# felixyu7/perceiver-io-1

Hardware: AMD Instinct MI355X
Metric: samples/sec (whole node) IMDB MLM seq_len=512 at 1/2/4/8 MI355X (higher is better)
Workload: dtype bf16; 1 GPU; mlm256; model=perceiver-io-mlm latents=256x64 layers=3x(1+6) vocab=10003, global_batch=64, seq_len=512, parallelism=dp1, backend=hip, graph=True, allreduce_in_graph=False, bucket_update=False

## Files before the change

perceiver_io_amd/csrc/binding.cpp:

```cpp
#include <torch/extension.h>
#include <ATen/hip/HIPContext.h>
#include <hip/hip_runtime.h>

#include "host_api.h"

#include <unordered_map>
#include <vector>

using torch::Tensor;
using OptT = c10::optional<Tensor>;

namespace {
hipStream_t stream() { return at::hip::getCurrentHIPStream(); }

#ifndef PIO_CHECKS
#define PIO_CHECKS 0
#endif
int64_t check_errors(bool reset) {
  return (int64_t)(pio::check_errors_elementwise(reset) | pio::check_errors_optim(reset) |
                   pio::check_errors_mlm_head(reset) | pio::check_errors_ce_head(reset) | pio::check_errors_topk_head(reset) |
                   pio::check_errors_rowgemm(reset) | pio::check_errors_pixel_head(reset) |
                   pio::check_errors_soft_ce_head(reset) | pio::check_errors_augment(reset) |
                   pio::check_errors_randaugment(reset) | pio::check_errors_health(reset) |
                   pio::check_errors_lartpc_prep(reset));
// ... 1365 lines not shown
}

Tensor embed_fwd(Tensor ids, Tensor E, Tensor P, double scale) {
  TORCH_CHECK(ids.is_contiguous() && E.is_contiguous() && P.is_contiguous());
  CHECK_DT(ids, torch::kInt64);
  const long long rows = ids.numel();
  const int L = (int)ids.size(1), C = (int)E.size(1);
  TORCH_CHECK(C % 4 == 0, "embedding width must be a multiple of 4");
  Tensor out = torch::empty({ids.size(0), L, C}, E.options());
  pio::embed_fwd_launch(ids.data_ptr<int64_t>(), f32p(E), f32p(P), out.data_ptr<float>(), rows, L, C, (float)scale,
                        E.size(0), stream());
  checked_sync("embed_fwd");
  return out;
}

void embed_bwd(Tensor ids, Tensor g, OptT dE, OptT dP, double scale, OptT job_slab, std::vector<Tensor> job_dsts,
               std::vector<int64_t> job_offs) {
  TORCH_CHECK(g.is_contiguous() && ids.is_contiguous());
  const pio::SlabJob job = make_job(job_slab, job_dsts, job_offs);
  const int B = (int)ids.size(0), L = (int)ids.size(1), C = (int)g.size(2);
  if (dE.has_value()) TORCH_CHECK(dE->is_contiguous() && dE->size(1) == C, "dE must be (V, C) contiguous");
  if (dP.has_value()) TORCH_CHECK(dP->is_contiguous() && dP->size(1) == C && dP->size(0) >= L, "dP must be (>= L, C)");
  if ((!dE.has_value() || dE->size(0) < (1 << 24)) &&
      pio::embed_bwd_local_launch(ids.data_ptr<int64_t>(), f32p(g), dE.has_value() ? dE->data_ptr<float>() : nullptr,
                                  dP.has_value() ? dP->data_ptr<float>() : nullptr, B, L, C, (float)scale, job,
                                  stream()))
    return;
  if (job.slab) pio::slab_reduce_launch(job, stream());
  if (dE.has_value()) {
    TORCH_CHECK(dE->is_contiguous() && dE->size(1) == C, "dE must be (V, C) contiguous");
// ... 827 lines not shown
        py::arg("w2"), py::arg("g2"), py::arg("be2"), py::arg("H"), py::arg("pa_grads"),
        py::arg("job_slab") = py::none(), py::arg("job_dsts") = std::vector<Tensor>(),
        py::arg("job_offs") = std::vector<int64_t>(), py::arg("seed") = py::none(), py::arg("site") = 0,
        py::arg("p") = 0.0, py::arg("zero_out") = py::none(), py::arg("att_qkv") = py::none(),
        py::arg("att_lse") = py::none(), py::arg("att_out") = py::none(), py::arg("att_scale") = 0.0);
  m.def("post_attn_bwd", &post_attn_bwd, py::arg("dz"), py::arg("y"), py::arg("m2"), py::arg("r2"), py::arg("u"),
        py::arg("o"), py::arg("wo"), py::arg("w1"), py::arg("w2"), py::arg("g2"), py::arg("be2"), py::arg("H"),
        py::arg("grads"), py::arg("slab") = false, py::arg("job_slab") = py::none(),
        py::arg("job_dsts") = std::vector<Tensor>(), py::arg("job_offs") = std::vector<int64_t>(),
        py::arg("seed") = py::none(), py::arg("site") = 0, py::arg("p") = 0.0, py::arg("zero_out") = py::none());
  m.def("ln_linear_bwd", &ln_linear_bwd, py::arg("g"), py::arg("w"), py::arg("x"), py::arg("mean"), py::arg("rstd"),
        py::arg("lnw"), py::arg("lnb"), py::arg("dres"), py::arg("need_dx"), py::arg("dlnw"), py::arg("dlnb"),
        py::arg("dW"), py::arg("db"), py::arg("pe") = py::none(), py::arg("kin") = -1, py::arg("slab") = false,
        py::arg("job_slab") = py::none(), py::arg("job_dsts") = std::vector<Tensor>(),
        py::arg("job_offs") = std::vector<int64_t>(), py::arg("dx_out") = py::none(), py::arg("pe_index") = py::none());
  m.def("wgrad", &wgrad, py::arg("g"), py::arg("a"), py::arg("amode"), py::arg("mean"), py::arg("rstd"), py::arg("lnw"),
        py::arg("lnb"), py::arg("rows_per_wg"), py::arg("dW"), py::arg("db"), py::arg("pe") = py::none(),
        py::arg("kin") = -1, py::arg("pe_index") = py::none());
  m.def("mlm_select", &mlm_select, py::arg("labels"), py::arg("cap"), py::arg("gcap"), py::arg("sticky") = py::none(),
        py::arg("queries") = py::none());
  m.def("index_add_rows", &index_add_rows);
  m.def("gather_rows", &gather_rows, py::arg("src"), py::arg("idx"));
  m.def("batch_sum2", &batch_sum2, py::arg("a"), py::arg("b"), py::arg("ob_acc") = py::none());
  m.def("pixel_ce_fwd", &pixel_ce_fwd);
  m.def("pixel_ce_bwd", &pixel_ce_bwd);
  m.def("pixel_predict", &pixel_predict, py::arg("h"), py::arg("w"), py::arg("b"), py::arg("qidx"), py::arg("qvalid"),
        py::arg("Q"), py::arg("npix"), py::arg("labels") = py::none());
  m.def("nonzero_compact", &nonzero_compact, py::arg("img"), py::arg("cap"), py::arg("segs") = 0, py::arg("tile") = 0);
  m.def("event_compact", &event_compact, py::arg("img"), py::arg("lab"), py::arg("words"), py::arg("key_cap"),
        py::arg("query_cap"), py::arg("wmask"), py::arg("ncls"), py::arg("segs") = 0, py::arg("tile") = 0);
// ... 76 lines not shown
```

perceiver_io_amd/csrc/host_api.h:

```cpp
#pragma once
#include <stdint.h>

#include <hip/hip_runtime_api.h>

namespace pio {


struct AttnArgs {
  const uint16_t* q; long long q_bs; int q_rs;
  const uint16_t* k; long long k_bs; int k_rs;
  const uint16_t* v; long long v_bs; int v_rs;
  const uint8_t* kmask;
  int B, H, Nq, Nk;
  float scale_log2;
  float scale;
  uint32_t drop_thresh;
  float drop_scale;
  const int64_t* seedp;
  uint32_t site;
};

struct DropCfg {
  const int64_t* seed;
  uint32_t site;
// ... 93 lines not shown
  RowsOut Y;
  float *mean, *rstd;
  PeSplit ps;
};
struct LnLinearBwdArgs {
  RowsIn G; int N;
  const uint16_t* W; int w_rs, Kin;
  RowsIn X;
  const float *mean, *rstd, *lnw, *lnb;
  const float* dres; int dres_rs;
  float* dX; int dx_rs;
  float *dlnw, *dlnb, *dW, *db;
  int vrs, wrs, slab;
  int R;
  PeSplit ps;
  SlabJob job;
};
struct WgradArgs {
  RowsIn G; int N;
  RowsIn A; int Kin, amode;
  const float *mean, *rstd, *lnw, *lnb;
  int R;
  int rows_per_wg;
  float *dW, *db;
  int vrs, wrs;
  PeSplit ps;
};
struct PostAttnFwdArgs {
  const uint16_t* O;
  const float* X;
// ... 194 lines not shown
                          uint8_t* classes, float* conf, uint8_t* cmap, int* cpart, hipStream_t st);
void nonzero_compact_launch(const float* img, int B, long long npix, long long cap, int S, int V, int* segcount,
                            float* values, int64_t* index, bool* kmask, int* count, hipStream_t st);
unsigned check_errors_pixel_head(bool reset);
void rand_augment_launch(const uint8_t* src, const float* words, uint8_t* out, uint8_t* tmp, int* hist, int B, int H,
                         int W, int C, int N, int fill, hipStream_t st);
unsigned check_errors_randaugment(bool reset);
void ln_linear_fwd_launch(const LnLinearFwdArgs& a, hipStream_t st);
void post_attn_fwd_launch(const PostAttnFwdArgs& a, int C, hipStream_t st);
void post_attn_ln_linear_fwd_launch(const PostAttnFwdArgs& a, int C, hipStream_t st);
bool sa_layer_fwd_launch(const SaLayerFwdArgs& a, hipStream_t st);
void post_attn_bwd_launch(const PostAttnBwdArgs& a, int C, hipStream_t st);
bool ln_linear_post_attn_bwd_launch(const LnLinearPostAttnBwdArgs& a, int C, hipStream_t st);
void ln_linear_bwd_launch(const LnLinearBwdArgs& a, hipStream_t st);
void wgrad_launch(const WgradArgs& a, hipStream_t st);
unsigned check_errors_rowgemm(bool reset);
bool sb_fwd_launch(const SBFwdArgs& a, int C, hipStream_t st);
bool sb_bwd_launch(const SBBwdArgs& a, int C, hipStream_t st);
bool sb_wgrad_launch(SBWgradArgs a, int C, const SlabJob& sj, hipStream_t st);
int soft_ce_row_tiles(int M);
void soft_ce_fwd_launch(int C, const float* Hm, const uint16_t* W, const float* bias, const int64_t* la,
                        const int64_t* lb, const float* lam, float eps, int M, int V, float* lse, int* pred,
                        uint16_t* hs, float* blk, float* loss, float* count, hipStream_t st);
void soft_ce_bwd_launch(int C, const uint16_t* Hs, const uint16_t* W, const float* bias, const int64_t* la,
                        const int64_t* lb, const float* lam, float eps, const float* lse, const float* gout,
                        const float* count, int M, int V, float* dH, float* dW, float* db, int accumulate,
                        hipStream_t st);
void batch_mix_launch(const float* x, const int64_t* y, const float* mix, float* out, int64_t* yb, float* lam_out, int B,
                      int H, int W, int Ch, hipStream_t st);
unsigned check_errors_soft_ce_head(bool reset);
// ... 9 lines not shown
```

perceiver_io_amd/csrc/rowgemm.hip:

```cpp
#include "common.h"

namespace pio {

__device__ __forceinline__ float ldf(const float* p) { return *p; }
__device__ __forceinline__ float ldf(const uint16_t* p) { return bf2f(*p); }
__device__ __forceinline__ void stf(float* p, float v) { *p = v; }
__device__ __forceinline__ void stf(uint16_t* p, float v) { *p = f2bf(v); }

template <int MAXT, bool A_KC, bool B_KC>
__device__ __forceinline__ void tile_gemm(const uint16_t* sA, int lda, const uint16_t* sB, int ldb, int BM, int BN,
                                          int K, f32x16 (&acc)[MAXT]) {
  const int w = wave_id();
  const int ntn = BN / 32, nt = (BM / 32) * ntn;
#pragma unroll
  for (int t = 0; t < MAXT; ++t) {
    const int tg = w + 4 * t;
    if (tg < nt) {
      const int m0 = 32 * (tg / ntn), n0 = 32 * (tg % ntn);
      for (int k0 = 0; k0 < K; k0 += 16) {
        const bf16x8 a = A_KC ? frag_kc(sA, lda, m0, k0) : frag_ks(sA, lda, m0, k0);
        const bf16x8 b = B_KC ? frag_kc(sB, ldb, n0, k0) : frag_ks(sB, ldb, n0, k0);
        acc[t] = mfma32(a, b, acc[t]);
      }
    }
// ... 318 lines not shown
    }
  }
}
__device__ __forceinline__ void g_store(const float (&v)[2][8], uint16_t* sG, int ldg) {
#pragma unroll
  for (int i = 0; i < 2; ++i) {
    bf16x8 b;
#pragma unroll
    for (int e = 0; e < 8; ++e) b[e] = (short)f2bf(v[i][e]);
    *reinterpret_cast<bf16x8*>(sG + ((threadIdx.x >> 3) + 32 * i) * ldg + (threadIdx.x & 7) * 8) = b;
  }
}

template <int NCH>
constexpr int ln_linear_fwd_smem() { return 2 * 64 * (32 * NCH + 8) * 2 + 64 * 68 * 4; }

template <typename TOut, int NCH, bool AV>
__device__ __forceinline__ void ln_linear_fwd_tile(float (&xv)[NCH][8], bf16x8 (&wb)[NCH], const float (&gw)[NCH][8],
                                                   const float (&gb)[NCH][8], bool has_ln, int m0, int R, int Kin,
                                                   float eps, const uint16_t* __restrict__ W, int w_rs,
                                                   const float* __restrict__ bias, int N, int act,
                                                   const float* __restrict__ res, int res_rs, TOut* __restrict__ Y,
                                                   int y_rs, float* __restrict__ mean_out, float* __restrict__ rstd_out,
                                                   uint16_t* smem, int part = 0, int nparts = 1, bool wv = false) {
  constexpr int KP = 32 * NCH, LD = KP + 8, LDO = 64 + 4;
  uint16_t* sA = smem;
  uint16_t* sW = sA + 64 * LD;
  float* sO = reinterpret_cast<float*>(sW + 64 * LD);
  const int gr = m0 + rp_row(), w = wave_id(), l = lane_id();
  const bool wvec = AV || wv;
  const int wk = w_rs > Kin ? w_rs : Kin;
  const bool yvec = (N & 7) == 0 && (y_rs & 7) == 0 && aligned16(Y);
  if (has_ln) {
    float s = 0.f;
#pragma unroll
    for (int j = 0; j < NCH; ++j)
#pragma unroll
      for (int e = 0; e < 8; ++e) s += xv[j][e];
    const float mean = quad_sum(s) / Kin;
    float q = 0.f;
#pragma unroll
    for (int j = 0; j < NCH; ++j)
#pragma unroll
      for (int e = 0; e < 8; ++e) {
        const float d = rp_col(j) + e < Kin ? xv[j][e] - mean : 0.f;
        q += d * d;
      }
    const float rstd = rsqrtf(quad_sum(q) / Kin + eps);
    if ((threadIdx.x & 3) == 0 && gr < R && mean_out && part == nparts - 1) { mean_out[gr] = mean; rstd_out[gr] = rstd; }
#pragma unroll
    for (int j = 0; j < NCH; ++j)
#pragma unroll
      for (int e = 0; e < 8; ++e) xv[j][e] = (xv[j][e] - mean) * rstd * gw[j][e] + gb[j][e];
  }
  lds_row_write_bf16<NCH>(sA, LD, xv);

  for (int n0 = 64 * part; n0 < N; n0 += 64 * nparts) {
    tile_store<NCH>(wb, sW, LD, 64, KP);
    lds_sync();
    if (n0 + 64 * nparts < N) tile_fetch<NCH>(wb, W, w_rs, n0 + 64 * nparts, N, 64, wk, KP, wvec);
    const int bc = n0 + 32 * (w & 1) + (l & 31);
    const float bv = (bias && bc < N) ? bias[bc] : 0.f;
    f32x16 acc[1] = {f32x16{}};
    tile_gemm<1, true, true>(sA, LD, sW, LD, 64, 64, KP, acc);
    for_acc<1>(64, 64, [&](int t, int m, int n, int i) {
      float v = acc[t][i] + bv;
      if (act == 1) v = gelu_f(v);
      sO[m * LDO + n] = v;
// ... 505 lines not shown
  post_attn_bwd_body<C, AV>(dz, Ysave, mean2, rstd2, U, O, Wo, W1, W2, g2, be2, dY, dO, delta, H, gr_out, R, dr, smem,
                            (int)blockIdx.y, (int)gridDim.y);
}

template <int NCH>
constexpr int ln_linear_bwd_loop_smem() {
  return 64 * 72 * 2 + 2 * 64 * (32 * NCH + 8) * 2 > 64 * (32 * NCH + 4) * 4
             ? 64 * 72 * 2 + 2 * 64 * (32 * NCH + 8) * 2
             : 64 * (32 * NCH + 4) * 4;
}
template <int NCH>
constexpr int ln_linear_bwd_smem() {
  return ln_linear_bwd_loop_smem<NCH>() + 8 * 32 * NCH * 4 + 4 * 64 * 4;
}

template <typename TG, typename TX, int NCH, bool AV>
__device__ __forceinline__ void ln_linear_bwd_body(
    const TG* __restrict__ G, int g_rs, int N, const uint16_t* __restrict__ W, int w_rs, int Kin,
    const TX* __restrict__ X,
    int x_rs, const float* __restrict__ mean, const float* __restrict__ rstd, const float* __restrict__ lnw,
    const float* __restrict__ lnb, const float* __restrict__ dres, int dres_rs, float* __restrict__ dX, int dx_rs,
    float* __restrict__ dlnw, float* __restrict__ dlnb, float* __restrict__ dW, float* __restrict__ db, int vrs,
    int wrs, int slab, int R, PeSplit ps, uint16_t* smem, float (&dxo)[NCH][8], int part = 0, int nparts = 1,
    int vf = 0) {
  const bool own_rows = tile_part_owner(3, nparts) == part;
  constexpr int KP = 32 * NCH, LD = KP + 8, LDG = 64 + 8, LDF = KP + 4;
  uint16_t* sG = smem;
  uint16_t* sW = sG + 64 * LDG;
  uint16_t* sXn = sW + 64 * LD;
  float* sF = reinterpret_cast<float*>(smem);
// ... 25 lines not shown
#pragma unroll
        for (int e = 0; e < 8; ++e) xn[j][e] += (xv[j][e] - mu) * rs * gw[j][e];
    } else {
#pragma unroll
      for (int j = 0; j < NCH; ++j)
#pragma unroll
        for (int e = 0; e < 8; ++e) xn[j][e] = xv[j][e];
    }
    lds_row_write_bf16<NCH>(sXn, LD, xn);
  }

  constexpr int MAXT = 3;
  f32x16 acc[MAXT];
#pragma unroll
  for (int t = 0; t < MAXT; ++t) acc[t] = f32x16{};
  for (int nc = 0; nc < N; nc += 64) {
    g_store(gv, sG, LDG);
    tile_store<NCH>(wb, sW, LD, 64, KP);
    float cs[8];
#pragma unroll
    for (int e = 0; e < 8; ++e) cs[e] = gv[0][e] + gv[1][e];
    lds_sync();
    if (nc + 64 < N) {
      g_fetch<TG>(gv, G, g_rs, m0, R, nc + 64, N, gvec);
      tile_fetch<NCH>(wb, W, w_rs, nc + 64, N, 64, wk, KP, wvec);
    }
    tile_gemm<MAXT, true, false>(sG, LDG, sW, LD, 64, KP, 64, acc);
    const bool mine = (nc >> 6) % nparts == part;
    if (dW && mine) {
      wgrad_tile<MAXT>(sG, LDG, sXn, LD, 64, KP, N - nc, Kin, rep(dW, wrs, slab) + (long long)nc * Kin, Kin, slab);
      if (db) {
#pragma unroll
        for (int e = 0; e < 8; ++e) {
          const float s = xor32_sum(xor16_sum(cs[e] + dpp<0x128>(cs[e])));
          if (l < 8) sPb[w * 64 + 8 * l + e] = s;
        }
      }
    }
    lds_sync();
    if (dW && mine && db && threadIdx.x < 64 && nc + (int)threadIdx.x < N) {
      const int t = threadIdx.x;
      gadd(rep(db, vrs, slab) + nc + t, sPb[t] + sPb[64 + t] + sPb[128 + t] + sPb[192 + t], slab);
    }
  }
  for_acc<MAXT>(64, KP, [&](int t, int m, int n, int i) { sF[m * LDF + n] = acc[t][i]; });
  lds_sync();

  float dr[NCH][8];
  if (dres) row_load<NCH>(dr, dres, dres_rs, gr, R, Kin, AV);
  float dxn[NCH][8];
  lds_row_read<NCH>(dxn, sF, LDF);
  if (lnw) {
    float s1 = 0.f, s2 = 0.f;
#pragma unroll
    for (int j = 0; j < NCH; ++j)
#pragma unroll
      for (int e = 0; e < 8; ++e) {
        xv[j][e] = rp_col(j) + e < Kin ? (xv[j][e] - mu) * rs : 0.f;
        const float g = dxn[j][e] * gw[j][e];
// ... 157 lines not shown
    const int gn = n0 + m;
    if (gn < N && n < Kin) atomicAdd(dWr + (long long)gn * Kin + n, acc[t][i]);
  });
  if (db) {
#pragma unroll
    for (int e = 0; e < 8; ++e) {
      const float v = xor32_sum(xor16_sum(cs[e] + dpp<0x128>(cs[e])));
      if (l < 8) sPb[w * 64 + 8 * l + e] = v;
    }
    lds_sync();
    if (threadIdx.x < 64 && n0 + (int)threadIdx.x < N) {
      const int t = threadIdx.x;
      atomicAdd(rep(db, vrs, 0) + n0 + t, sPb[t] + sPb[64 + t] + sPb[128 + t] + sPb[192 + t]);
    }
  }
}

static void set_smem_once(const void* fn) {
  static const void* done[256] = {nullptr};
  for (auto& d : done) {
    if (d == fn) return;
    if (d == nullptr) {
      (void)hipFuncSetAttribute(fn, hipFuncAttributeMaxDynamicSharedMemorySize, 160 * 1024);
      d = fn;
      return;
    }
  }
}

static bool al16(const void* p) { return (reinterpret_cast<uintptr_t>(p) & 15) == 0; }
// ... 201 lines not shown
void wgrad_launch(const WgradArgs& a, hipStream_t st) {
  const int nblk = (a.N + 63) / 64;
  int rps = a.rows_per_wg;
  if (rps <= 0) {
    const int splits = (512 + nblk - 1) / nblk;
    rps = (a.R + splits - 1) / splits;
  }
  rps = round_up(rps < 64 ? 64 : rps, 64);
  const int nch = pick_nch(a.Kin);
  if (a.G.bf16 && a.A.bf16) wgrad_n<uint16_t, uint16_t>(nch, a, rps, st);
  else if (a.G.bf16) wgrad_n<uint16_t, float>(nch, a, rps, st);
  else if (a.A.bf16) wgrad_n<float, uint16_t>(nch, a, rps, st);
  else wgrad_n<float, float>(nch, a, rps, st);
}

}

namespace pio {
unsigned check_errors_rowgemm(bool reset) { return pio_read_errors(reset); }
}
```

perceiver_io_amd/ops/emulation.py:

```python
from __future__ import annotations

import math
import torch
import torch.nn.functional as F

LOG2E = 1.4426950408889634


def _bf(x):
    return x.to(torch.bfloat16).to(torch.float32)


M32 = 0xFFFFFFFF


def _u32(x):
    return x & M32


def hash3(a, b, c):
    h = _u32(_u32(a * 0x9E3779B1) ^ _u32(b + 0x7F4A7C15))
    h = h ^ _u32(c * 0x85EBCA77)
    h = _u32((h ^ (h >> 15)) * 0x2C1B3C6D)
    h = _u32((h ^ (h >> 12)) * 0x297A2D39)
# ... 712 lines not shown
    B = src.shape[0]
    w = words.detach().to(device=src.device, dtype=torch.float32)
    out = torch.empty_like(src)
    for b in range(B):
        x = src[b].to(torch.int64)
        for l in range(w.shape[1]):
            x = _ra_layer(x, w[b, l], fill)
        out[b] = x.to(torch.uint8)
    return out


def embed_fwd(ids, E, P, scale):
    return E[ids] * scale + P[: ids.shape[1]].unsqueeze(0)


def embed_bwd(ids, g, dE, dP, scale, job_slab=None, job_dsts=(), job_offs=()):
    _run_job(job_slab, job_dsts, job_offs)
    C = g.shape[-1]
    if dE is not None:
        dE.index_add_(0, ids.reshape(-1), g.reshape(-1, C) * scale)
    if dP is not None:
        dP[: ids.shape[1]] += g.sum(0)


def _unit24(h):
    return (h >> 8).to(torch.float32) * (1.0 / 16777216.0)


def _mulhi32(a, b: int):
    return ((a >> 16) * b + (((a & 0xFFFF) * b) >> 16)) >> 16
# ... 517 lines not shown
```

perceiver_io_amd/ops/fused.py:

```python
from __future__ import annotations

import math
import os
from dataclasses import dataclass
from typing import List, Optional

import torch

from . import emulation, ext
from ..parallel.reducer import bucket_ready_point

EPS = 1e-5
WGRAD_SLAB = True
BF16_DQKV = True
ATTN_SLAB = True
CHAIN_ATT = True
TALL_ROWS = 1 << 17


def kernels(t: torch.Tensor):
    return ext.require() if t.is_cuda else emulation


class WeightCache:
# ... 375 lines not shown
        xq2 = x_q.reshape(Bq * Nq, C)
        if not xq2.is_contiguous():
            xq2 = xq2.contiguous()
        if spec.cross:
            B, M = x_kv.shape[0], x_kv.shape[1]
            xkv2 = x_kv.reshape(B * M, x_kv.shape[2])
            hq = _LOOKAHEAD["have_q"]
            if hq is not None and hq[4] is g_q and hq[0].data_ptr() == xq2.data_ptr() and hq[0].numel() == xq2.numel():
                q, mean_q, rstd_q = hq[1:4]
                _LOOKAHEAD["have_q"] = None
                ctx.q_handoff = True
            else:
                q, mean_q, rstd_q = K.ln_linear_fwd(xq2, g_q, b_q, EPS, wq, bin_[:C], 0, None, True, True)
            key = id(ps[0])
            ent = src.entries.get(key) if src is not None else None
            ctx.kv_owner = ent is None
            if ent is None:
                kv_sb = False
                factored = (PE_FACTORED and src is not None and src.pe is not None and src.index is None
                            and not spec.packed
                            and not ctx.needs_input_grad[6] and 1 <= xkv2.shape[1] <= 4 and 2 * C <= 512)
                implicit = (factored and PE_IMPLICIT and PE_ATTN_FUSED and D == 32 and Nq <= 32 and kmask is None
                            and p_attn == 0.0 and hasattr(K, "attn_fwd_pe"))
                imp = None
                if implicit:
                    imp = _pe_implicit_operands(K, xkv2.shape[1], src.pe, g_kv, b_kv, (ps[5], ps[6]), bin_[C:])
                    kv = mean_kv = rstd_kv = None
                elif factored:
                    kv, mean_kv, rstd_kv = _pe_proj_fwd(K, xkv2, src.pe, g_kv, b_kv,
                                                        torch.cat([ps[5], ps[6]], 0), bin_[C:])
                else:
# ... 213 lines not shown
                sl = _GradSlab(Rq, [C, C, C * C, C], dz2)
                dx_q = K.ln_linear_bwd(dq2, wq, xq2, mean_q, rstd_q, g_q, b_q, dres, True, *sl.targets(), slab=True,
                                       **_take_job(), **q_out)
                sl.defer(K, [flat(g_q), flat(b_q), flat(ps[4], 0, C * C), flat(bin_, 0, C)])
            else:
                gwq = rows(gb(ps[4]), 0, C, C) if spec.packed else gb(ps[4])
                dx_q = K.ln_linear_bwd(dq2, wq, xq2, mean_q, rstd_q, g_q, b_q, dres, True, gb(g_q), gb(b_q), gwq,
                                       rows(gb(bin_), 0, C, 1), **q_out)
            dx_kv = None
            if ctx.kv_owner and ent.get("sb_bwd") and ent.get("pe_D") is None:
                _LOOKAHEAD["bwd_q"] = dict(key=xkv2.data_ptr(), g=dkv.view(B * M, 2 * C), dres=None,
                                           ll_dsts=[flat(g_kv), flat(b_kv), flat(ps[4], C * C, 3 * C * C),
                                                    flat(bin_, C, 3 * C)])
                dx_kv = _zero_stand_in(B * M, Ckv, dkv.device)
                ent["dkv"] = None
            elif ctx.kv_owner:
                if ent.get("pe_D") is not None:
                    dkv2, Rkv = None, B * M
                else:
                    dkv2 = dkv.view(B * M, 2 * C)
                    Rkv = dkv2.shape[0]
                if ent.get("factored"):
                    if ent.get("pe_D") is not None:
                        Dm, part = ent["pe_D"], ent["pe_part"]
                    else:
                        Dm, part = K.pe_proj_bwd(dkv2, xkv2, mean_kv, rstd_kv, M)
                    nc = xkv2.shape[1]
                    ebf = _pe_table(ctx.kv_pe, nc, g_kv.shape[0])[0]

                    def tg(p):
# ... 549 lines not shown
        return layer.eager_forward(x)
    return _run_layer(layer, x)


def cross_attention_layer(layer, x_q, x_kv, pad_mask=None):
    src = x_kv if isinstance(x_kv, KVSource) else None
    if not can_fuse(layer, x_kv):
        if src is not None:
            x_kv = src.materialize()
        return layer.eager_forward(x_q, x_kv, pad_mask)
    if x_q.dim() == 3 and x_q.shape[0] > 1 and x_q.stride(0) == 0:
        x_q = x_q[:1]
    return _run_layer(layer, x_q, src.x if src is not None else x_kv, pad_mask, src)


class _TextEmbedFn(torch.autograd.Function):
    @staticmethod
    def forward(ctx, ids, emb, pos, scale):
        K = kernels(emb)
        ids = ids.contiguous()
        out = K.embed_fwd(ids, emb, pos[: ids.shape[1]].contiguous(), scale)
        ctx.save_for_backward(ids)
        ctx.scale, ctx.emb, ctx.pos = scale, emb, pos
        return out

    @staticmethod
    def backward(ctx, g):
        (ids,) = ctx.saved_tensors
        K = kernels(g)
        targets = []
        for p, need in ((ctx.emb, ctx.needs_input_grad[1]), (ctx.pos, ctx.needs_input_grad[2])):
            if need and p.grad is None:
                p.grad = torch.zeros_like(p)
            targets.append(p.grad if need else None)
        from . import deterministic

        if deterministic() and g.is_cuda:
            C = g.shape[-1]
            if targets[0] is not None:
                targets[0].index_put_((ids.reshape(-1),), g.reshape(-1, C) * ctx.scale, accumulate=True)
            if targets[1] is not None:
                targets[1][: ids.shape[1]] += g.sum(0)
            return None, None, None, None
        K.embed_bwd(ids, g.contiguous(), targets[0], targets[1], ctx.scale, **_take_job())
        return None, None, None, None


def text_embed(adapter, ids):
    return _TextEmbedFn.apply(ids, adapter.text_embedding.weight, adapter.pos_encoding, float(adapter.scale))


def encoder_forward(encoder, x, pad_mask=None):
    from ..models.adapters import ImageInputAdapter, TextInputAdapter

    ad = encoder.input_adapter
    if isinstance(ad, TextInputAdapter):
        src = KVSource(text_embed(ad, x))
    elif isinstance(ad, ImageInputAdapter) and not x.requires_grad:
        ad.check_shape(x)
        pix = x.reshape(x.shape[0], -1, ad.num_image_channels).float().contiguous()
        src = KVSource(pix, pe=ad.padded_position_encoding(), kin=ad.num_input_channels)
    else:
        src = KVSource(ad(x))
    return _encode(encoder, src, pad_mask)


def encode_inputs(encoder, x_in, pad_mask=None):
    return _encode(encoder, KVSource(x_in.float().contiguous()), pad_mask)


def encode_sparse(encoder, values, index, pad_mask=None):
    ad = encoder.input_adapter
# ... 76 lines not shown
```

perceiver_io_amd/parallel/reducer.py:

```python
from __future__ import annotations

import os
from typing import Dict, Iterable, List, Optional, Tuple

import torch
import torch.distributed as dist

_ACTIVE: List["FlatGradReducer"] = []


class _ReadyFn(torch.autograd.Function):

    @staticmethod
    def forward(ctx, x, red, name):
        ctx.red, ctx.name = red, name
        return x.view_as(x)

    @staticmethod
    def backward(ctx, g):
        ctx.red.point_reached(ctx.name)
        return g, None, None


def ready_point_armed(module: torch.nn.Module, name: str) -> bool:
    return any(red.armed and red.owns_point(module, name) for red in _ACTIVE)


def bucket_ready_point(x: torch.Tensor, module: torch.nn.Module, name: str) -> torch.Tensor:
    if not _ACTIVE or not torch.is_grad_enabled() or not x.requires_grad:
        return x
    for red in reversed(_ACTIVE):
        if red.owns_point(module, name):
            if not red.armed:
                return x
            return _ReadyFn.apply(x, red, name)
    return x


def _capturing(device) -> bool:
    return device.type == "cuda" and torch.cuda.is_current_stream_capturing()
# ... 279 lines not shown
```

Baseline: 48660 samples/s.

## Fuse text embedding with both cross-attention LN+KV projections in one kernel

```diff
diff --git a/perceiver_io_amd/csrc/binding.cpp b/perceiver_io_amd/csrc/binding.cpp
--- a/perceiver_io_amd/csrc/binding.cpp
+++ b/perceiver_io_amd/csrc/binding.cpp
@@ -1403,6 +1403,95 @@
   return out;
 }
 
+std::vector<Tensor> text_kv_fwd(Tensor ids, Tensor E, Tensor P, double scale, double eps, std::vector<Tensor> la,
+                                std::vector<Tensor> lb) {
+  CHECK_CUDA(ids); CHECK_CUDA(E);
+  TORCH_CHECK(ids.dim() == 2 && ids.is_contiguous() && E.is_contiguous() && P.is_contiguous());
+  CHECK_DT(ids, torch::kInt64);
+  const int64_t B = ids.size(0), L = ids.size(1), R = B * L;
+  TORCH_CHECK(E.dim() == 2 && E.size(1) == 64 && P.dim() == 2 && P.size(1) == 64 && P.size(0) >= L,
+              "text_kv_fwd: 64-channel embedding and position tables, at least L positions");
+  TORCH_CHECK(R > 0 && R < (int64_t(1) << 31), "text_kv_fwd: bad row count");
+  TORCH_CHECK(la.size() == 4 && lb.size() == 4, "text_kv_fwd: [lnw, lnb, w, bias] per layer");
+  auto opts = E.options();
+  Tensor x = torch::empty({B, L, 64}, opts);
+  Tensor mean = torch::empty({R}, opts), rstd = torch::empty({R}, opts);
+  Tensor kva = torch::empty({R, 128}, opts.dtype(torch::kBFloat16)), kvb = torch::empty({R, 128}, opts.dtype(torch::kBFloat16));
+  auto proj = [](std::vector<Tensor>& l, Tensor& kv) {
+    TORCH_CHECK(l[0].is_contiguous() && l[0].numel() == 64 && l[1].is_contiguous() && l[1].numel() == 64,
+                "text_kv_fwd: LN affine of 64 channels");
+    TORCH_CHECK(l[2].dim() == 2 && l[2].is_contiguous() && l[2].size(0) == 128 && l[2].size(1) == 64,
+                "text_kv_fwd: w must be (128, 64) contiguous");
+    TORCH_CHECK(l[3].is_contiguous() && l[3].numel() == 128, "text_kv_fwd: bias of 128 columns");
+    return pio::TextKvProj{f32p(l[0]), f32p(l[1]), bfp(l[2]), f32p(l[3]), bfp_mut(kv)};
+  };
+  pio::TextKvFwdArgs a{};
+  a.ids = ids.data_ptr<int64_t>();
+  a.E = f32p(E);
+  a.P = f32p(P);
+  a.scale = (float)scale;
+  a.V = E.size(0);
+  a.L = (int)L;
+  a.R = (int)R;
+  a.eps = (float)eps;
+  a.a = proj(la, kva);
+  a.b = proj(lb, kvb);
+  a.X = x.data_ptr<float>();
+  a.mean = mean.data_ptr<float>();
+  a.rstd = rstd.data_ptr<float>();
+  TORCH_CHECK(pio::text_kv_fwd_launch(a, stream()), "text_kv_fwd: operands must be 16-byte aligned");
+  checked_sync("text_kv_fwd");
+  return {x, mean, rstd, kva, kvb};
+}
+
+Tensor text_kv_bwd(Tensor ga, Tensor gb, Tensor x, Tensor mean, Tensor rstd, std::vector<Tensor> la,
+                   std::vector<Tensor> lb, std::vector<Tensor> grads, bool slab, OptT job_slab,
+                   std::vector<Tensor> job_dsts, std::vector<int64_t> job_offs) {
+  CHECK_CUDA(ga); CHECK_CUDA(x);
+  const int64_t R = ga.size(0);
+  TORCH_CHECK(ga.dim() == 2 && ga.is_contiguous() && ga.size(1) == 128 && gb.is_contiguous() && gb.dim() == 2 &&
+                  gb.size(0) == R && gb.size(1) == 128,
+              "text_kv_bwd: dK|dV must be (R, 128) contiguous");
+  TORCH_CHECK(x.is_contiguous() && x.numel() == R * 64 && mean.is_contiguous() && mean.numel() == R &&
+                  rstd.is_contiguous() && rstd.numel() == R,
+              "text_kv_bwd: x (R, 64) and its row statistics");
+  TORCH_CHECK(R > 0 && R < kTallRows, "text_kv_bwd: bad row count");
+  TORCH_CHECK(!g_det || slab, "deterministic mode: text_kv_bwd parameter gradients need slab mode");
+  TORCH_CHECK(la.size() == 3 && lb.size() == 3 && grads.size() == 8, "text_kv_bwd: [lnw, lnb, w] per layer, 8 targets");
+  const int64_t sr = slab ? (R + 63) / 64 : 0;
+  int vrs = -1;
+  auto layer = [&](const Tensor& g, std::vector<Tensor>& l, int t0) {
+    TORCH_CHECK(l[0].is_contiguous() && l[0].numel() == 64 && l[1].is_contiguous() && l[1].numel() == 64,
+                "text_kv_bwd: LN affine of 64 channels");
+    TORCH_CHECK(l[2].dim() == 2 && l[2].is_contiguous() && l[2].size(0) == 128 && l[2].size(1) == 64,
+                "text_kv_bwd: w must be (128, 64) contiguous");
+    pio::TextKvGrad o{};
+    o.G = f32p(g);
+    o.lnw = f32p(l[0]);
+    o.lnb = f32p(l[1]);
+    o.W = bfp(l[2]);
+    o.dlnw = vec_target(grads[t0], 64, "dlnw", vrs, sr);
+    o.dlnb = vec_target(grads[t0 + 1], 64, "dlnb", vrs, sr);
+    o.dW = vec_target(grads[t0 + 2], 128 * 64, "dW", vrs, sr);
+    o.db = vec_target(grads[t0 + 3], 128, "db", vrs, sr);
+    return o;
+  };
+  Tensor dx = torch::empty({R, 64}, ga.options());
+  pio::TextKvBwdArgs a{};
+  a.a = layer(ga, la, 0);
+  a.b = layer(gb, lb, 4);
+  a.X = f32p(x);
+  a.mean = f32p(mean);
+  a.rstd = f32p(rstd);
+  a.dX = dx.data_ptr<float>();
+  a.vrs = vrs < 0 ? 0 : vrs;
+  a.slab = slab ? 1 : 0;
+  a.R = (int)R;
+  a.job = make_job(job_slab, job_dsts, job_offs);
+  TORCH_CHECK(pio::text_kv_bwd_launch(a, stream()), "text_kv_bwd: operands must be 16-byte aligned");
+  return dx;
+}
+
 void embed_bwd(Tensor ids, Tensor g, OptT dE, OptT dP, double scale, OptT job_slab, std::vector<Tensor> job_dsts,
                std::vector<int64_t> job_offs) {
   TORCH_CHECK(g.is_contiguous() && ids.is_contiguous());
@@ -2260,6 +2349,11 @@
         py::arg("dW"), py::arg("db"), py::arg("pe") = py::none(), py::arg("kin") = -1, py::arg("slab") = false,
         py::arg("job_slab") = py::none(), py::arg("job_dsts") = std::vector<Tensor>(),
         py::arg("job_offs") = std::vector<int64_t>(), py::arg("dx_out") = py::none(), py::arg("pe_index") = py::none());
+  m.def("text_kv_fwd", &text_kv_fwd, py::arg("ids"), py::arg("E"), py::arg("P"), py::arg("scale"), py::arg("eps"),
+        py::arg("la"), py::arg("lb"));
+  m.def("text_kv_bwd", &text_kv_bwd, py::arg("ga"), py::arg("gb"), py::arg("x"), py::arg("mean"), py::arg("rstd"),
+        py::arg("la"), py::arg("lb"), py::arg("grads"), py::arg("slab") = false, py::arg("job_slab") = py::none(),
+        py::arg("job_dsts") = std::vector<Tensor>(), py::arg("job_offs") = std::vector<int64_t>());
   m.def("wgrad", &wgrad, py::arg("g"), py::arg("a"), py::arg("amode"), py::arg("mean"), py::arg("rstd"), py::arg("lnw"),
         py::arg("lnb"), py::arg("rows_per_wg"), py::arg("dW"), py::arg("db"), py::arg("pe") = py::none(),
         py::arg("kin") = -1, py::arg("pe_index") = py::none());
diff --git a/perceiver_io_amd/csrc/host_api.h b/perceiver_io_amd/csrc/host_api.h
--- a/perceiver_io_amd/csrc/host_api.h
+++ b/perceiver_io_amd/csrc/host_api.h
@@ -131,6 +131,35 @@
   int vrs, wrs, slab;
   int R;
   PeSplit ps;
+  SlabJob job;
+};
+struct TextKvProj {
+  const float *lnw, *lnb;
+  const uint16_t* W;
+  const float* bias;
+  uint16_t* KV;
+};
+struct TextKvFwdArgs {
+  const int64_t* ids;
+  const float *E, *P;
+  float scale;
+  long long V;
+  int L, R;
+  float eps;
+  TextKvProj a, b;
+  float *X, *mean, *rstd;
+};
+struct TextKvGrad {
+  const float* G;
+  const float *lnw, *lnb;
+  const uint16_t* W;
+  float *dlnw, *dlnb, *dW, *db;
+};
+struct TextKvBwdArgs {
+  TextKvGrad a, b;
+  const float *X, *mean, *rstd;
+  float* dX;
+  int vrs, slab, R;
   SlabJob job;
 };
 struct WgradArgs {
@@ -355,6 +384,8 @@
 bool ln_linear_post_attn_bwd_launch(const LnLinearPostAttnBwdArgs& a, int C, hipStream_t st);
 void ln_linear_bwd_launch(const LnLinearBwdArgs& a, hipStream_t st);
 void wgrad_launch(const WgradArgs& a, hipStream_t st);
+bool text_kv_fwd_launch(const TextKvFwdArgs& a, hipStream_t st);
+bool text_kv_bwd_launch(const TextKvBwdArgs& a, hipStream_t st);
 unsigned check_errors_rowgemm(bool reset);
 bool sb_fwd_launch(const SBFwdArgs& a, int C, hipStream_t st);
 bool sb_bwd_launch(const SBBwdArgs& a, int C, hipStream_t st);
diff --git a/perceiver_io_amd/csrc/rowgemm.hip b/perceiver_io_amd/csrc/rowgemm.hip
--- a/perceiver_io_amd/csrc/rowgemm.hip
+++ b/perceiver_io_amd/csrc/rowgemm.hip
@@ -356,6 +356,28 @@
 
 template <int NCH>
 constexpr int ln_linear_fwd_smem() { return 2 * 64 * (32 * NCH + 8) * 2 + 64 * 68 * 4; }
+
+template <int NCH>
+__device__ __forceinline__ void ln_row_stats(const float (&xv)[NCH][8], int Kin, float eps, float& mean, float& rstd) {
+  float s = 0.f;
+#pragma unroll
+  for (int j = 0; j < NCH; ++j)
+#pragma unroll
+    for (int e = 0; e < 8; ++e) s += xv[j][e];
+  mean = quad_sum(s) / Kin;
+  float q = 0.f;
+#pragma unroll
+  for (int j = 0; j < NCH; ++j)
+#pragma unroll
+    for (int e = 0; e < 8; ++e) {
+      const float d = rp_col(j) + e < Kin ? xv[j][e] - mean : 0.f;
+      q = __builtin_fmaf(d, d, q);
+    }
+  rstd = rsqrtf(quad_sum(q) / Kin + eps);
+}
+__device__ __forceinline__ float ln_affine(float x, float mean, float rstd, float g, float b) {
+  return __builtin_fmaf((x - mean) * rstd, g, b);
+}
 
 template <typename TOut, int NCH, bool AV>
 __device__ __forceinline__ void ln_linear_fwd_tile(float (&xv)[NCH][8], bf16x8 (&wb)[NCH], const float (&gw)[NCH][8],
@@ -374,26 +396,13 @@
   const int wk = w_rs > Kin ? w_rs : Kin;
   const bool yvec = (N & 7) == 0 && (y_rs & 7) == 0 && aligned16(Y);
   if (has_ln) {
-    float s = 0.f;
+    float mean, rstd;
+    ln_row_stats<NCH>(xv, Kin, eps, mean, rstd);
+    if ((threadIdx.x & 3) == 0 && gr < R && mean_out && part == nparts - 1) { mean_out[gr] = mean; rstd_out[gr] = rstd; }
 #pragma unroll
     for (int j = 0; j < NCH; ++j)
 #pragma unroll
-      for (int e = 0; e < 8; ++e) s += xv[j][e];
-    const float mean = quad_sum(s) / Kin;
-    float q = 0.f;
-#pragma unroll
-    for (int j = 0; j < NCH; ++j)
-#pragma unroll
-      for (int e = 0; e < 8; ++e) {
-        const float d = rp_col(j) + e < Kin ? xv[j][e] - mean : 0.f;
-        q += d * d;
-      }
-    const float rstd = rsqrtf(quad_sum(q) / Kin + eps);
-    if ((threadIdx.x & 3) == 0 && gr < R && mean_out && part == nparts - 1) { mean_out[gr] = mean; rstd_out[gr] = rstd; }
-#pragma unroll
-    for (int j = 0; j < NCH; ++j)
-#pragma unroll
-      for (int e = 0; e < 8; ++e) xv[j][e] = (xv[j][e] - mean) * rstd * gw[j][e] + gb[j][e];
+      for (int e = 0; e < 8; ++e) xv[j][e] = ln_affine(xv[j][e], mean, rstd, gw[j][e], gb[j][e]);
   }
   lds_row_write_bf16<NCH>(sA, LD, xv);
 
@@ -929,6 +938,47 @@
   return ln_linear_bwd_loop_smem<NCH>() + 8 * 32 * NCH * 4 + 4 * 64 * 4;
 }
 
+template <typename TG, int NCH, int MAXT>
+__device__ __forceinline__ void ln_linear_bwd_chunks(float (&gv)[2][8], bf16x8 (&wb)[NCH], f32x16 (&acc)[MAXT],
+                                                     const TG* __restrict__ G, int g_rs, int N,
+                                                     const uint16_t* __restrict__ W, int w_rs, int wk, int Kin, int m0,
+                                                     int R, bool gvec, bool wvec, uint16_t* sG, uint16_t* sW,
+                                                     const uint16_t* sXn, float* sPb, float* __restrict__ dW,
+                                                     float* __restrict__ db, int vrs, int wrs, int slab, int part,
+                                                     int nparts) {
+  constexpr int KP = 32 * NCH, LD = KP + 8, LDG = 64 + 8;
+  const int w = wave_id(), l = lane_id();
+  for (int nc = 0; nc < N; nc += 64) {
+    g_store(gv, sG, LDG);
+    tile_store<NCH>(wb, sW, LD, 64, KP);
+    float cs[8];
+#pragma unroll
+    for (int e = 0; e < 8; ++e) cs[e] = gv[0][e] + gv[1][e];
+    lds_sync();
+    if (nc + 64 < N) {
+      g_fetch<TG>(gv, G, g_rs, m0, R, nc + 64, N, gvec);
+      tile_fetch<NCH>(wb, W, w_rs, nc + 64, N, 64, wk, KP, wvec);
+    }
+    tile_gemm<MAXT, true, false>(sG, LDG, sW, LD, 64, KP, 64, acc);
+    const bool mine = (nc >> 6) % nparts == part;
+    if (dW && mine) {
+      wgrad_tile<MAXT>(sG, LDG, sXn, LD, 64, KP, N - nc, Kin, rep(dW, wrs, slab) + (long long)nc * Kin, Kin, slab);
+      if (db) {
+#pragma unroll
+        for (int e = 0; e < 8; ++e) {
+          const float s = xor32_sum(xor16_sum(cs[e] + dpp<0x128>(cs[e])));
+          if (l < 8) sPb[w * 64 + 8 * l + e] = s;
+        }
+      }
+    }
+    lds_sync();
+    if (dW && mine && db && threadIdx.x < 64 && nc + (int)threadIdx.x < N) {
+      const int t = threadIdx.x;
+      gadd(rep(db, vrs, slab) + nc + t, sPb[t] + sPb[64 + t] + sPb[128 + t] + sPb[192 + t], slab);
+    }
+  }
+}
+
 template <typename TG, typename TX, int NCH, bool AV>
 __device__ __forceinline__ void ln_linear_bwd_body(
     const TG* __restrict__ G, int g_rs, int N, const uint16_t* __restrict__ W, int w_rs, int Kin,
@@ -984,35 +1034,8 @@
   f32x16 acc[MAXT];
 #pragma unroll
   for (int t = 0; t < MAXT; ++t) acc[t] = f32x16{};
-  for (int nc = 0; nc < N; nc += 64) {
-    g_store(gv, sG, LDG);
-    tile_store<NCH>(wb, sW, LD, 64, KP);
-    float cs[8];
-#pragma unroll
-    for (int e = 0; e < 8; ++e) cs[e] = gv[0][e] + gv[1][e];
-    lds_sync();
-    if (nc + 64 < N) {
-      g_fetch<TG>(gv, G, g_rs, m0, R, nc + 64, N, gvec);
-      tile_fetch<NCH>(wb, W, w_rs, nc + 64, N, 64, wk, KP, wvec);
-    }
-    tile_gemm<MAXT, true, false>(sG, LDG, sW, LD, 64, KP, 64, acc);
-    const bool mine = (nc >> 6) % nparts == part;
-    if (dW && mine) {
-      wgrad_tile<MAXT>(sG, LDG, sXn, LD, 64, KP, N - nc, Kin, rep(dW, wrs, slab) + (long long)nc * Kin, Kin, slab);
-      if (db) {
-#pragma unroll
-        for (int e = 0; e < 8; ++e) {
-          const float s = xor32_sum(xor16_sum(cs[e] + dpp<0x128>(cs[e])));
-          if (l < 8) sPb[w * 64 + 8 * l + e] = s;
-        }
-      }
-    }
-    lds_sync();
-    if (dW && mine && db && threadIdx.x < 64 && nc + (int)threadIdx.x < N) {
-      const int t = threadIdx.x;
-      gadd(rep(db, vrs, slab) + nc + t, sPb[t] + sPb[64 + t] + sPb[128 + t] + sPb[192 + t], slab);
-    }
-  }
+  ln_linear_bwd_chunks<TG, NCH, MAXT>(gv, wb, acc, G, g_rs, N, W, w_rs, wk, Kin, m0, R, gvec, wvec, sG, sW, sXn, sPb, dW,
+                                      db, vrs, wrs, slab, part, nparts);
   for_acc<MAXT>(64, KP, [&](int t, int m, int n, int i) { sF[m * LDF + n] = acc[t][i]; });
   lds_sync();
 
@@ -1200,6 +1223,167 @@
       atomicAdd(rep(db, vrs, 0) + n0 + t, sPb[t] + sPb[64 + t] + sPb[128 + t] + sPb[192 + t]);
     }
   }
+}
+
+__global__ __launch_bounds__(256) void text_kv_fwd_kernel(const int64_t* __restrict__ ids, const float* __restrict__ E,
+                                                          const float* __restrict__ P, float scale, long long V, int L,
+                                                          int R, float eps, TextKvProj pa, TextKvProj pb,
+                                                          float* __restrict__ X, float* __restrict__ mean_out,
+                                                          float* __restrict__ rstd_out) {
+  constexpr int NCH = 2, C = 64, N = 128;
+  extern __shared__ __attribute__((aligned(16))) uint16_t smem[];
+  const int m0 = blockIdx.x * 64, gr = m0 + rp_row();
+  long long id = ids[gr < R ? gr : R - 1];
+#if PIO_CHECKS
+  if (id < 0 || id >= V) {
+    pio_flag(kErrEmbedId);
+    id = id < 0 ? 0 : V - 1;
+  }
+#else
+  (void)V;
+#endif
+  bf16x8 wa[NCH], wb[NCH];
+  tile_fetch<NCH>(wa, pa.W, C, 0, N, 64, C, C, true);
+  tile_fetch<NCH>(wb, pb.W, C, 0, N, 64, C, C, true);
+  float ga[NCH][8], ba[NCH][8], gb[NCH][8], bb[NCH][8];
+  row_load<NCH>(ga, pa.lnw, 0, 0, 1, C, true);
+  row_load<NCH>(ba, pa.lnb, 0, 0, 1, C, true);
+  row_load<NCH>(gb, pb.lnw, 0, 0, 1, C, true);
+  row_load<NCH>(bb, pb.lnb, 0, 0, 1, C, true);
+  float xv[NCH][8], pv[NCH][8];
+#pragma unroll
+  for (int j = 0; j < NCH; ++j) {
+    const float* e = E + id * C + rp_col(j);
+    const float* p = P + (long long)((gr < R ? gr : R - 1) % L) * C + rp_col(j);
+    const float4 e0 = *reinterpret_cast<const float4*>(e), e1 = *reinterpret_cast<const float4*>(e + 4);
+    const float4 p0 = *reinterpret_cast<const float4*>(p), p1 = *reinterpret_cast<const float4*>(p + 4);
+    xv[j][0] = e0.x; xv[j][1] = e0.y; xv[j][2] = e0.z; xv[j][3] = e0.w;
+    xv[j][4] = e1.x; xv[j][5] = e1.y; xv[j][6] = e1.z; xv[j][7] = e1.w;
+    pv[j][0] = p0.x; pv[j][1] = p0.y; pv[j][2] = p0.z; pv[j][3] = p0.w;
+    pv[j][4] = p1.x; pv[j][5] = p1.y; pv[j][6] = p1.z; pv[j][7] = p1.w;
+  }
+#pragma unroll
+  for (int j = 0; j < NCH; ++j)
+#pragma unroll
+    for (int e = 0; e < 8; ++e) xv[j][e] = __builtin_fmaf(xv[j][e], scale, pv[j][e]);
+  row_store<NCH>(xv, X, C, gr, R, C, true);
+  float mean, rstd;
+  ln_row_stats<NCH>(xv, C, eps, mean, rstd);
+  if ((threadIdx.x & 3) == 0 && gr < R) { mean_out[gr] = mean; rstd_out[gr] = rstd; }
+  float av[NCH][8];
+#pragma unroll
+  for (int j = 0; j < NCH; ++j)
+#pragma unroll
+    for (int e = 0; e < 8; ++e) av[j][e] = ln_affine(xv[j][e], mean, rstd, ga[j][e], ba[j][e]);
+  ln_linear_fwd_tile<uint16_t, NCH, true>(av, wa, ga, ba, false, m0, R, C, eps, pa.W, C, pa.bias, N, 0, nullptr, 0, pa.KV,
+                                          N, nullptr, nullptr, smem);
+#pragma unroll
+  for (int j = 0; j < NCH; ++j)
+#pragma unroll
+    for (int e = 0; e < 8; ++e) av[j][e] = ln_affine(xv[j][e], mean, rstd, gb[j][e], bb[j][e]);
+  ln_linear_fwd_tile<uint16_t, NCH, true>(av, wb, gb, bb, false, m0, R, C, eps, pb.W, C, pb.bias, N, 0, nullptr, 0, pb.KV,
+                                          N, nullptr, nullptr, smem);
+}
+
+constexpr int text_kv_bwd_smem() { return 4 * 64 * 72 * 2 + 16 * 64 * 4 + 4 * 64 * 4; }
+
+__global__ __launch_bounds__(256) void text_kv_bwd_kernel(TextKvGrad la, TextKvGrad lb, const float* __restrict__ X,
+                                                          const float* __restrict__ mean,
+                                                          const float* __restrict__ rstd, float* __restrict__ dX, int vrs,
+                                                          int slab, int R, SlabJob job) {
+  constexpr int NCH = 2, C = 64, N = 128, KP = 64, LD = KP + 8, LDG = 64 + 8, LDF = KP + 4;
+  extern __shared__ __attribute__((aligned(16))) uint16_t smem[];
+  if ((int)blockIdx.x >= (R + 63) / 64) {
+    const int jb = (int)blockIdx.x - (R + 63) / 64;
+    if (jb < job.nblk) slab_reduce_block(job, jb, reinterpret_cast<float4*>(smem));
+    return;
+  }
+  uint16_t* sG = smem;
+  uint16_t* sW = sG + 64 * LDG;
+  uint16_t* sXa = sW + 64 * LD;
+  uint16_t* sXb = sXa + 64 * LD;
+  float* sFa = reinterpret_cast<float*>(sG);
+  float* sFb = reinterpret_cast<float*>(sXa);
+  float* sPart = reinterpret_cast<float*>(sXb + 64 * LD);
+  float* sPb = sPart + 16 * KP;
+  const int m0 = blockIdx.x * 64, gr = m0 + rp_row();
+
+  float xv[NCH][8], ga[NCH][8], gb[NCH][8];
+  row_load<NCH>(xv, X, C, gr, R, C, true);
+  const float mu = *(gr < R ? mean + gr : kZero32B);
+  const float rs = *(gr < R ? rstd + gr : kZero32B);
+  row_load<NCH>(ga, la.lnw, 0, 0, 1, C, true);
+  row_load<NCH>(gb, lb.lnw, 0, 0, 1, C, true);
+  float gva[2][8], gvb[2][8];
+  bf16x8 wa[NCH], wb[NCH];
+  g_fetch<float>(gva, la.G, N, m0, R, 0, N, true);
+  tile_fetch<NCH>(wa, la.W, C, 0, N, 64, C, KP, true);
+  g_fetch<float>(gvb, lb.G, N, m0, R, 0, N, true);
+  tile_fetch<NCH>(wb, lb.W, C, 0, N, 64, C, KP, true);
+  {
+    float xn[NCH][8];
+    row_load<NCH>(xn, la.lnb, 0, 0, 1, C, true);
+#pragma unroll
+    for (int j = 0; j < NCH; ++j)
+#pragma unroll
+      for (int e = 0; e < 8; ++e) xn[j][e] += (xv[j][e] - mu) * rs * ga[j][e];
+    lds_row_write_bf16<NCH>(sXa, LD, xn);
+    row_load<NCH>(xn, lb.lnb, 0, 0, 1, C, true);
+#pragma unroll
+    for (int j = 0; j < NCH; ++j)
+#pragma unroll
+      for (int e = 0; e < 8; ++e) xn[j][e] += (xv[j][e] - mu) * rs * gb[j][e];
+    lds_row_write_bf16<NCH>(sXb, LD, xn);
+  }
+
+  f32x16 acca[1] = {f32x16{}}, accb[1] = {f32x16{}};
+  ln_linear_bwd_chunks<float, NCH, 1>(gva, wa, acca, la.G, N, N, la.W, C, C, C, m0, R, true, true, sG, sW, sXa, sPb, la.dW,
+                                      la.db, vrs, vrs, slab, 0, 1);
+  ln_linear_bwd_chunks<float, NCH, 1>(gvb, wb, accb, lb.G, N, N, lb.W, C, C, C, m0, R, true, true, sG, sW, sXb, sPb, lb.dW,
+                                      lb.db, vrs, vrs, slab, 0, 1);
+  for_acc<1>(64, KP, [&](int t, int m, int n, int i) {
+    sFa[m * LDF + n] = acca[t][i];
+    sFb[m * LDF + n] = accb[t][i];
+  });
+  lds_sync();
+
+  float da[NCH][8], db_[NCH][8];
+  lds_row_read<NCH>(da, sFa, LDF);
+  lds_row_read<NCH>(db_, sFb, LDF);
+  float s1 = 0.f, s2 = 0.f;
+#pragma unroll
+  for (int j = 0; j < NCH; ++j)
+#pragma unroll
+    for (int e = 0; e < 8; ++e) {
+      xv[j][e] = (xv[j][e] - mu) * rs;
+      const float g = da[j][e] * ga[j][e] + db_[j][e] * gb[j][e];
+      ga[j][e] = g;
+      s1 += g;
+      s2 += g * xv[j][e];
+    }
+  s1 = quad_sum(s1) / C;
+  s2 = quad_sum(s2) / C;
+#pragma unroll
+  for (int j = 0; j < NCH; ++j)
+#pragma unroll
+    for (int e = 0; e < 8; ++e) ga[j][e] = rs * (ga[j][e] - s1 - xv[j][e] * s2);
+  row_store<NCH>(ga, dX, C, gr, R, C, true);
+  colsum_partial<NCH>(da, sPart + 4 * KP, KP);
+  colsum_partial<NCH>(db_, sPart + 12 * KP, KP);
+#pragma unroll
+  for (int j = 0; j < NCH; ++j)
+#pragma unroll
+    for (int e = 0; e < 8; ++e) {
+      da[j][e] *= xv[j][e];
+      db_[j][e] *= xv[j][e];
+    }
+  colsum_partial<NCH>(da, sPart, KP);
+  colsum_partial<NCH>(db_, sPart + 8 * KP, KP);
+  lds_sync();
+  colsum_flush(sPart, KP, rep(la.dlnw, vrs, slab), C, slab);
+  colsum_flush(sPart + 4 * KP, KP, rep(la.dlnb, vrs, slab), C, slab);
+  colsum_flush(sPart + 8 * KP, KP, rep(lb.dlnw, vrs, slab), C, slab);
+  colsum_flush(sPart + 12 * KP, KP, rep(lb.dlnb, vrs, slab), C, slab);
 }
 
 static void set_smem_once(const void* fn) {
@@ -1431,6 +1615,23 @@
   else wgrad_n<float, float>(nch, a, rps, st);
 }
 
+bool text_kv_fwd_launch(const TextKvFwdArgs& a, hipStream_t st) {
+  if (a.R <= 0 || a.L <= 0 ||
+      !av_ok({a.E, a.P, a.X, a.a.lnw, a.a.lnb, a.a.W, a.a.KV, a.b.lnw, a.b.lnb, a.b.W, a.b.KV}, {}))
+    return false;
+  hipLaunchKernelGGL(text_kv_fwd_kernel, dim3((a.R + 63) / 64), dim3(256), ln_linear_fwd_smem<2>(), st, a.ids, a.E, a.P,
+                     a.scale, a.V, a.L, a.R, a.eps, a.a, a.b, a.X, a.mean, a.rstd);
+  return true;
+}
+
+bool text_kv_bwd_launch(const TextKvBwdArgs& a, hipStream_t st) {
+  if (a.R <= 0 || !av_ok({a.a.G, a.a.lnw, a.a.lnb, a.a.W, a.b.G, a.b.lnw, a.b.lnb, a.b.W, a.X, a.dX}, {})) return false;
+  const dim3 grid((a.R + 63) / 64 + (a.job.slab ? a.job.nblk : 0));
+  hipLaunchKernelGGL(text_kv_bwd_kernel, grid, dim3(256), text_kv_bwd_smem(), st, a.a, a.b, a.X, a.mean, a.rstd, a.dX,
+                     a.vrs, a.slab, a.R, a.job);
+  return true;
+}
+
 }
 
 namespace pio {
diff --git a/perceiver_io_amd/ops/emulation.py b/perceiver_io_amd/ops/emulation.py
--- a/perceiver_io_amd/ops/emulation.py
+++ b/perceiver_io_amd/ops/emulation.py
@@ -750,6 +750,36 @@
     return E[ids] * scale + P[: ids.shape[1]].unsqueeze(0)
 
 
+def text_kv_fwd(ids, E, P, scale, eps, la, lb):
+    x = embed_fwd(ids, E, P, scale)
+    x2 = x.reshape(-1, x.shape[-1])
+    kva, mean, rstd = ln_linear_fwd(x2, la[0], la[1], eps, la[2], la[3], 0, None, True, True)
+    kvb = ln_linear_fwd(x2, lb[0], lb[1], eps, lb[2], lb[3], 0, None, True, False)[0]
+    return [x, mean, rstd, kva, kvb]
+
+
+def text_kv_bwd(ga, gb, x, mean, rstd, la, lb, grads, slab=False, job_slab=None, job_dsts=(), job_offs=()):
+    _run_job(job_slab, job_dsts, job_offs)
+    _SLAB[0] = slab
+    try:
+        xf = x.reshape(-1, x.shape[-1]).float()
+        xh = (xf - mean[:, None]) * rstd[:, None]
+        g = None
+        for G, (lnw, lnb, w), (dlnw, dlnb, dW, db) in ((ga, la, grads[0:4]), (gb, lb, grads[4:8])):
+            gf = G.float()
+            dxn = _bf(gf) @ _bf(w.float())
+            _acc(dW, _bf(gf).t() @ _bf(xh * lnw + lnb))
+            _acc(db, gf.sum(0))
+            _acc(dlnw, (dxn * xh).sum(0))
+            _acc(dlnb, dxn.sum(0))
+            g = dxn * lnw if g is None else g + dxn * lnw
+        s1 = g.mean(-1, keepdim=True)
+        s2 = (g * xh).mean(-1, keepdim=True)
+        return rstd[:, None] * (g - s1 - xh * s2)
+    finally:
+        _SLAB[0] = False
+
+
 def embed_bwd(ids, g, dE, dP, scale, job_slab=None, job_dsts=(), job_offs=()):
     _run_job(job_slab, job_dsts, job_offs)
     C = g.shape[-1]
diff --git a/perceiver_io_amd/ops/fused.py b/perceiver_io_amd/ops/fused.py
--- a/perceiver_io_amd/ops/fused.py
+++ b/perceiver_io_amd/ops/fused.py
@@ -413,7 +413,7 @@
                 q, mean_q, rstd_q = K.ln_linear_fwd(xq2, g_q, b_q, EPS, wq, bin_[:C], 0, None, True, True)
             key = id(ps[0])
             ent = src.entries.get(key) if src is not None else None
-            ctx.kv_owner = ent is None
+            ctx.kv_owner = ent is None or bool(ent.pop("claim", False))
             if ent is None:
                 kv_sb = False
                 factored = (PE_FACTORED and src is not None and src.pe is not None and src.index is None
@@ -657,6 +657,8 @@
                                                     flat(bin_, C, 3 * C)])
                 dx_kv = _zero_stand_in(B * M, Ckv, dkv.device)
                 ent["dkv"] = None
+            elif ctx.kv_owner and ent.get("tkv") is not None:
+                dx_kv = _text_kv_backward(K, ent, id(ps[0]), xkv2, mean_kv, rstd_kv, dz2)
             elif ctx.kv_owner:
                 if ent.get("pe_D") is not None:
                     dkv2, Rkv = None, B * M
@@ -1236,12 +1238,21 @@
     return _run_layer(layer, x_q, src.x if src is not None else x_kv, pad_mask, src)
 
 
+TEXT_KV_FUSED = os.environ.get("PERCEIVER_TEXT_KV_FUSED", "1") != "0"
+TEXT_KV_C = 64
+
+
 class _TextEmbedFn(torch.autograd.Function):
     @staticmethod
-    def forward(ctx, ids, emb, pos, scale):
+    def forward(ctx, ids, emb, pos, scale, kvp=None):
         K = kernels(emb)
         ids = ids.contiguous()
-        out = K.embed_fwd(ids, emb, pos[: ids.shape[1]].contiguous(), scale)
+        if kvp is not None:
+            C = TEXT_KV_C
+            la, lb = ([ps[2], ps[3], wkv, ps[5][C:]] for ps, wkv in kvp["layers"])
+            out, *kvp["out"] = K.text_kv_fwd(ids, emb, pos[: ids.shape[1]].contiguous(), scale, EPS, la, lb)
+        else:
+            out = K.embed_fwd(ids, emb, pos[: ids.shape[1]].contiguous(), scale)
         ctx.save_for_backward(ids)
         ctx.scale, ctx.emb, ctx.pos = scale, emb, pos
         return out
@@ -1263,21 +1274,87 @@
                 targets[0].index_put_((ids.reshape(-1),), g.reshape(-1, C) * ctx.scale, accumulate=True)
             if targets[1] is not None:
                 targets[1][: ids.shape[1]] += g.sum(0)
-            return None, None, None, None
+            return None, None, None, None, None
         K.embed_bwd(ids, g.contiguous(), targets[0], targets[1], ctx.scale, **_take_job())
-        return None, None, None, None
+        return None, None, None, None, None
 
 
 def text_embed(adapter, ids):
     return _TextEmbedFn.apply(ids, adapter.text_embedding.weight, adapter.pos_encoding, float(adapter.scale))
 
 
+def _text_kv_layers(encoder, ad, ids):
+    from . import deterministic
+
+    C = TEXT_KV_C
+    emb = ad.text_embedding.weight
+    if not (TEXT_KV_FUSED and WGRAD_SLAB) or deterministic() or not hasattr(kernels(emb), "text_kv_fwd"):
+        return None
+    layers = list(encoder.layers())
+    if len(layers) < 2 or any(l[0] is not layers[1][0] for l in layers[2:]) or layers[0][0] is layers[1][0]:
+        return None
+    if (ids.dim() != 2 or ids.dtype != torch.int64 or ids.numel() == 0 or ids.numel() >= TALL_ROWS
+            or emb.shape[1] != C or emb.dtype != torch.float32):
+        return None
+    from ..parallel.reducer import reducer_active
+
+    if reducer_active():
+        return None
+    out = []
+    for cross in (layers[0][0], layers[1][0]):
+        if not _fusable(cross):
+            return None
+        spec, ps = layer_spec_and_params(cross)
+        if not (spec.cross and spec.packed and spec.C == C and ps[2].shape[0] == C):
+            return None
+        out.append((ps, _bf16_weights(spec, ps)[1]))
+    return out
+
+
+def _text_kv_source(ad, ids, layers) -> KVSource:
+    kvp = {"layers": layers}
+    x = _TextEmbedFn.apply(ids, ad.text_embedding.weight, ad.pos_encoding, float(ad.scale), kvp)
+    mean, rstd, kva, kvb = kvp.pop("out")
+    src = KVSource(x)
+    tk = {"first": id(layers[0][0][0]), "layers": layers}
+    for (ps, wkv), kv in zip(layers, (kva, kvb)):
+        src.entries[id(ps[0])] = {"kv": kv, "mean": mean, "rstd": rstd, "dkv": None, "factored": False, "wkv": wkv,
+                                  "implicit": None, "sb_bwd": False, "tkv": tk, "claim": True}
+    tk["ents"] = tuple(src.entries[id(ps[0])] for ps, _ in layers)
+    return src
+
+
+def _text_kv_backward(K, ent, key, x2, mean, rstd, like):
+    tk = ent["tkv"]
+    if key != tk["first"]:
+        return None
+    ea, eb = tk["ents"]
+    if ea["dkv"] is None or eb["dkv"] is None:
+        raise RuntimeError("fused encoder: the text input backward needs the key/value gradients of both layer_1 "
+                           "and layer_n")
+    C = TEXT_KV_C
+    R = x2.shape[0]
+    sl = _GradSlab(R, [C, C, 2 * C * C, 2 * C] * 2, like)
+    ops, dsts = [], []
+    for ps, wkv in tk["layers"]:
+        ops.append([ps[2].detach(), ps[3].detach(), wkv])
+        flat = [None if _grad_of(p) is None else _grad_of(p).view(-1) for p in (ps[2], ps[3], ps[4], ps[5])]
+        dsts += [flat[0], flat[1], None if flat[2] is None else flat[2][C * C:3 * C * C],
+                 None if flat[3] is None else flat[3][C:3 * C]]
+    dx = K.text_kv_bwd(ea["dkv"].view(R, 2 * C), eb["dkv"].view(R, 2 * C), x2, mean, rstd, ops[0], ops[1],
+                       sl.targets(), slab=True, **_take_job())
+    sl.defer(K, dsts)
+    ea["dkv"] = eb["dkv"] = None
+    return dx
+
+
 def encoder_forward(encoder, x, pad_mask=None):
     from ..models.adapters import ImageInputAdapter, TextInputAdapter
 
     ad = encoder.input_adapter
     if isinstance(ad, TextInputAdapter):
-        src = KVSource(text_embed(ad, x))
+        kv_layers = _text_kv_layers(encoder, ad, x)
+        src = _text_kv_source(ad, x, kv_layers) if kv_layers is not None else KVSource(text_embed(ad, x))
     elif isinstance(ad, ImageInputAdapter) and not x.requires_grad:
         ad.check_shape(x)
         pix = x.reshape(x.shape[0], -1, ad.num_image_channels).float().contiguous()
diff --git a/perceiver_io_amd/parallel/reducer.py b/perceiver_io_amd/parallel/reducer.py
--- a/perceiver_io_amd/parallel/reducer.py
+++ b/perceiver_io_amd/parallel/reducer.py
@@ -24,6 +24,10 @@
 
 def ready_point_armed(module: torch.nn.Module, name: str) -> bool:
     return any(red.armed and red.owns_point(module, name) for red in _ACTIVE)
+
+
+def reducer_active() -> bool:
+    return bool(_ACTIVE)
 
 
 def bucket_ready_point(x: torch.Tensor, module: torch.nn.Module, name: str) -> torch.Tensor:
```

After: 49500 samples/s (median of 6 runs). 1.02x the previous value.
